# evo-design/evo

Hardware: AMD Instinct MI355X
Metric: nucleotides/sec forward scoring, evo-1 7B (higher is better)
Workload: dtype bf16; 1 GPU; evo-1-8k-base scoring, batch 8 x 8,192 nt per GPU (BASELINE configs[1]); batch_per_gpu=8, nt=8192, parallelism=single GPU

## Files before the change

### evo_amd/_build.py

```python
from __future__ import annotations

import os
import shutil
import subprocess
from pathlib import Path

ROOT = Path(__file__).resolve().parent
CSRC = ROOT / "csrc"
LIBDIR = ROOT / "_lib"
LIBNAME = os.environ.get("EVO_AMD_LIBNAME", "libevo_mi355x.so")
ARCH = "gfx950"

EXPORTS = [
    "evo_abi_version", "evo_embed_bf16", "evo_rmsnorm_bf16", "evo_hyena_seg_state", "evo_hyena_carry_scan", "evo_hyena_carry_add",
    "evo_hyena_apply", "evo_hyena_step", "evo_rope_qk_bf16", "evo_attn_fwd_causal_bf16", "evo_attn_decode_bf16",
    "evo_linear_small_m_bf16", "evo_mlp_gate_small_m_bf16", "evo_norm_mlp_gate_small_m_bf16", "evo_norm_linear_small_m_bf16", "evo_hyena_decode_fused_small_m", "evo_linear_mfma_bf16", "evo_mlp_gate_mfma_bf16", "evo_linear_xblk_mfma_bf16", "evo_hyena_ct", "evo_linear_t_mfma_bf16", "evo_rmsnorm_rows_bf16", "evo_gelu_gate_bf16",
    "evo_logprob_entropy", "evo_unembed_logprob_bf16", "evo_unembed_profile_bf16", "evo_rope_append_decode_bf16",
    "evo_linear_mfma_nf_bf16", "evo_linear_xblk_mfma_nf_bf16", "evo_mlp_gate_mfma_nf_bf16", "evo_linear_t_mfma_nf_bf16", "evo_rms_finalize_f32",
    "evo_probe_copy_f4", "evo_probe_mfma_bf16", "evo_pool_rows_bf16", "evo_sample_rows_f32",
    "evo_attn_fwd_prefix_bf16", "evo_attn_prefix_vt_bf16", "evo_attn_decode_prefix_bf16", "evo_rope_append_decode_at_bf16",
    "evo_hyena_state_at_zt",
]


def lib_path() -> Path:
    return LIBDIR / LIBNAME


def sources():
    return sorted(CSRC.glob("*.hip"))


def _hipcc() -> str:
    for cand in (os.environ.get("HIPCC"), shutil.which("hipcc"), "/opt/rocm/bin/hipcc"):
        if cand and os.path.exists(cand):
            return cand
    raise RuntimeError("hipcc not found: cannot build libevo_mi355x.so")


def is_stale() -> bool:
    out = lib_path()
    if not out.exists():
        return True
    deps = list(sources()) + list(CSRC.glob("*.h")) + [ROOT.parent / "include" / "evo_mi355x.h"]
    newest = max(p.stat().st_mtime for p in deps if p.exists())
    return newest > out.stat().st_mtime


FILE_FLAGS = {"attn_w64.hip": ["-fno-slp-vectorize", "-Wno-unused-value"]}


def _compile_one(args):
    src, obj, verbose = args
    cmd = [_hipcc(), f"--offload-arch={ARCH}", "-O3", "-std=c++17", "-fPIC", "-fno-gpu-rdc", "-Wno-inline-asm"] \
# ... 37 lines not shown
```

### evo_amd/ops.py

```python
from __future__ import annotations

import ctypes
import math
import os
import threading
from typing import Optional, Tuple

import torch

from . import _build

_c = ctypes
_PTR = _c.c_void_p
_I64 = _c.c_int64
_F32 = _c.c_float

_SIGNATURES = {
    "evo_abi_version": ([], _c.c_int),
    "evo_embed_bf16": ([_PTR, _PTR, _PTR, _I64, _I64, _I64, _PTR, _PTR], _c.c_int),
    "evo_rmsnorm_bf16": ([_PTR, _PTR, _PTR, _PTR, _I64, _I64, _F32, _PTR], _c.c_int),
    "evo_hyena_seg_state": ([_PTR, _PTR, _PTR, _PTR, _PTR, _PTR, _PTR, _I64, _I64, _I64, _I64, _I64, _PTR], _c.c_int),
    "evo_hyena_carry_scan": ([_PTR, _PTR, _PTR, _PTR, _I64, _I64, _I64, _I64, _PTR], _c.c_int),
    "evo_hyena_carry_add": ([_PTR, _PTR, _PTR, _I64, _I64, _I64, _I64, _PTR], _c.c_int),
    "evo_hyena_apply": ([_PTR] * 10 + [_I64] * 5 + [_PTR], _c.c_int),
# ... 1 lines not shown
    "evo_rope_qk_bf16": ([_PTR, _PTR, _PTR, _I64, _I64, _I64, _I64, _F32, _PTR], _c.c_int),
    "evo_attn_fwd_causal_bf16": ([_PTR] * 4 + [_I64] * 14 + [_F32, _PTR, _PTR], _c.c_int),
    "evo_attn_fwd_prefix_bf16": ([_PTR] * 6 + [_I64] * 16 + [_F32, _PTR, _PTR], _c.c_int),
    "evo_attn_prefix_vt_bf16": ([_PTR] * 2 + [_I64] * 5 + [_PTR], _c.c_int),
    "evo_attn_decode_bf16": ([_PTR] * 4 + [_I64] * 11 + [_PTR] * 3 + [_I64, _F32, _PTR], _c.c_int),
    "evo_linear_small_m_bf16": ([_PTR] * 5 + [_I64] * 3 + [_PTR, _I64, _PTR], _c.c_int),
    "evo_linear_mfma_bf16": ([_PTR] * 5 + [_I64] * 3 + [_PTR], _c.c_int),
    "evo_mlp_gate_mfma_bf16": ([_PTR] * 3 + [_I64] * 3 + [_PTR], _c.c_int),
    "evo_hyena_ct": ([_PTR] * 9 + [_I64] * 13 + [_PTR], _c.c_int),
    "evo_linear_t_mfma_bf16": ([_PTR] * 4 + [_I64] * 3 + [_PTR], _c.c_int),
    "evo_rmsnorm_rows_bf16": ([_PTR, _PTR, _PTR, _PTR, _I64, _I64, _F32, _I64, _I64, _I64, _I64, _PTR], _c.c_int),
    "evo_linear_xblk_mfma_bf16": ([_PTR] * 5 + [_I64] * 3 + [_PTR], _c.c_int),
    "evo_linear_mfma_nf_bf16": ([_PTR] * 7 + [_I64] * 4 + [_PTR], _c.c_int),
    "evo_linear_xblk_mfma_nf_bf16": ([_PTR] * 6 + [_I64] * 4 + [_PTR], _c.c_int),
    "evo_mlp_gate_mfma_nf_bf16": ([_PTR] * 4 + [_I64] * 3 + [_PTR], _c.c_int),
    "evo_linear_t_mfma_nf_bf16": ([_PTR] * 5 + [_I64] * 6 + [_PTR], _c.c_int),
    "evo_rms_finalize_f32": ([_PTR, _I64, _I64, _PTR, _I64, _I64, _I64, _F32, _PTR, _PTR], _c.c_int),
    "evo_probe_copy_f4": ([_PTR, _PTR, _I64, _PTR], _c.c_int),
    "evo_probe_mfma_bf16": ([_PTR, _I64, _I64, _PTR], _c.c_int),
    "evo_mlp_gate_small_m_bf16": ([_PTR] * 3 + [_I64] * 4 + [_PTR], _c.c_int),
    "evo_norm_linear_small_m_bf16": ([_PTR] * 5 + [_I64] * 3 + [_c.c_float, _PTR], _c.c_int),
    "evo_norm_mlp_gate_small_m_bf16": ([_PTR] * 4 + [_I64] * 3 + [_c.c_float, _I64, _PTR], _c.c_int),
    "evo_hyena_decode_fused_small_m": ([_PTR] * 12 + [_I64] * 3 + [_c.c_float, _PTR], _c.c_int),
    "evo_gelu_gate_bf16": ([_PTR, _PTR, _I64, _I64, _PTR], _c.c_int),
    "evo_logprob_entropy": ([_PTR, _I64, _PTR, _PTR, _PTR, _I64, _I64, _PTR], _c.c_int),
    "evo_unembed_logprob_bf16": ([_PTR] * 5 + [_I64] * 3 + [_PTR], _c.c_int),
    "evo_unembed_profile_bf16": ([_PTR] * 3 + [_c.POINTER(_c.c_int32), _I64] + [_PTR] * 3 + [_I64] * 3 + [_PTR], _c.c_int),
    "evo_rope_append_decode_bf16": ([_PTR] * 4 + [_F32] + [_I64] * 7 + [_F32, _PTR], _c.c_int),
    "evo_pool_rows_bf16": ([_PTR, _I64, _I64, _I64, _PTR, _I64, _PTR, _F32, _I64, _I64, _PTR, _PTR, _PTR], _c.c_int),
    "evo_attn_decode_prefix_bf16": ([_PTR] * 4 + [_I64] * 11 + [_PTR] * 3 + [_I64] * 8 + [_PTR] * 4 + [_I64, _I64, _F32, _PTR], _c.c_int),
    "evo_rope_append_decode_at_bf16": ([_PTR] * 4 + [_F32] + [_I64] * 7 + [_F32, _PTR, _PTR], _c.c_int),
    "evo_hyena_state_at_zt": ([_PTR] * 8 + [_I64] * 8 + [_PTR], _c.c_int),
    "evo_sample_rows_f32": ([_PTR, _I64, _I64, _PTR, _PTR, _PTR, _PTR, _c.c_uint64] + [_PTR] * 7 + [_I64] * 3 + [_PTR], _c.c_int),
}

_LIB = None
ABI_VERSION = 16
ATTN_GROUP_ROWS = 8


HYENA_RAGGED_SEG = 256


class EvoLibraryError(RuntimeError):
    pass


def load_library(build_if_missing: bool = True) -> ctypes.CDLL:
    global _LIB
    if _LIB is not None:
        return _LIB
    path = _build.lib_path()
    if (not path.exists() or (_build.is_stale() and os.environ.get("EVO_AMD_NO_REBUILD") != "1")) and build_if_missing:
        try:
            _build.build()
        except Exception as e:
            if not path.exists():
                raise EvoLibraryError(f"libevo_mi355x.so is missing and could not be built: {e}") from e
            import warnings
            warnings.warn(f"{path} is older than its sources and the rebuild failed ({e}); loading the stale library "
                          f"(its ABI version is checked below)")
    if not path.exists():
        raise EvoLibraryError(f"{path} not found; run `python -c 'import __graft_entry__ as g; g.build()'`")
    lib = ctypes.CDLL(str(path))
    for name, (argtypes, restype) in _SIGNATURES.items():
        fn = getattr(lib, name, None)
        if fn is None:
            raise EvoLibraryError(f"{path} does not export {name}")
        fn.argtypes = argtypes
        fn.restype = restype
# ... 45 lines not shown

    def span(self, name):
        return KernelTimer._Span(self, name)

    def summary(self):
        return {k: (len(v), sum(a.elapsed_time(b) for a, b in v) / len(v)) for k, v in self.pairs.items()}


class _NoSpan:
    def __enter__(self):
        return None

    def __exit__(self, *exc):
        return False


_NOSPAN = _NoSpan()


class HipOps:

    name = "hip-gfx950"

    def __init__(self):
        self.lib = load_library()
        if not torch.cuda.is_available():
            raise EvoLibraryError("HipOps needs a ROCm GPU (torch.cuda.is_available() is False)")
        self.seg_len_override = int(os.environ.get("EVO_AMD_SEG_LEN", "0"))
        self.attn_gemm_mfma = True
        self.attn_w64 = True
        self.fuse_norm = True
        self.attn_prescale = True
        self.hyena_tail_split = True
        self.gate_small_m_mfma = True
        self.hyena_table_guard = True
        self.all_gemm_mfma = True
        self.mlp_gate_fused = True
        self.timer: Optional[KernelTimer] = None
        self.validate_ids = os.environ.get("EVO_AMD_VALIDATE_IDS", "1") != "0"
        self.hyena_mfma = True
        self.hyena_ct_flag = True
        self._xpad = threading.local()
        self.last_hyena_io = {}

    def _t(self, name):
        return self.timer.span(name) if self.timer is not None else _NOSPAN

    PTR_ALIGN = 16

    @staticmethod
    def _align_of(dtype) -> int:
        return HipOps.PTR_ALIGN if (dtype.is_floating_point or dtype.is_complex) else torch.empty(0, dtype=dtype).element_size()

    @staticmethod
    def _check_address(addr: int, what: str, align: int = 16) -> None:
        if addr % align:
            raise RuntimeError(f"{what}: address 0x{addr:x} is not {align}-byte aligned (include/evo_mi355x.h, Conventions)")

    @staticmethod
    def _need(t: torch.Tensor, dtype, what: str):
        if not t.is_cuda:
            raise RuntimeError(f"{what}: tensor is on {t.device}; the HIP path has no CPU fallback")
        if t.dtype != dtype:
            raise RuntimeError(f"{what}: expected {dtype}, got {t.dtype}")
        if not t.is_contiguous():
            raise RuntimeError(f"{what}: tensor must be contiguous")
# ... 190 lines not shown
        Tm, Tp, Mp, r = self.zt_layout(B, T)
        K = xp.shape[1]
        N = w.shape[0]
        assert xp.shape[0] >= Mp + B * r
        zt = torch.empty(Mp // 256 + (1 if r and tail else 0), N, 256, dtype=torch.bfloat16, device=xp.device)
        self._launch("gemm_zt", "evo_linear_t_mfma_bf16", xp.data_ptr(), w.data_ptr(), _ptr(b), zt.data_ptr(), Mp, N, K)
        if r and tail:
            self._zt_tail_fill(zt, self._linear_small_m(xp[Mp:Mp + B * r], w, b, None), B, r)
        return zt

    @staticmethod
    def _zt_tail_fill(zt: torch.Tensor, z_tail: torch.Tensor, B: int, r: int) -> None:
        N = zt.shape[1]
        zt[-1].zero_()
        zt[-1].view(N, 32, 8)[:, :B, :r] = z_tail.view(B, r, N).permute(2, 0, 1)

    @staticmethod
    def zt_rows(zt: torch.Tensor, B: int, T: int, t0: int, n: int) -> torch.Tensor:
        bb = torch.arange(B, device=zt.device)[:, None].expand(B, n)
        tt = torch.arange(t0, t0 + n, device=zt.device)[None, :].expand(B, n)
        pos = HipOps.zt_positions(B, T, bb, tt).reshape(-1)
        return zt[pos // 256, :, pos % 256].view(B, n, zt.shape[1])

    @staticmethod
    def zt_from_rows(z: torch.Tensor, B: int, T: int, pad_value: float = 0.0) -> torch.Tensor:
        Tm, Tp, Mp, r = HipOps.zt_layout(B, T)
        C = z.shape[-1]
        P = Mp + (256 if r else 0)
        flat = torch.full((C, P), pad_value, dtype=z.dtype, device=z.device)
        flat[:, :B * Tp].view(C, B, Tp)[:, :, :Tm] = z[:, :Tm].permute(2, 0, 1)
        if r:
            flat[:, Mp:].view(C, 32, 8)[:, :B, :r] = z[:, Tm:].permute(2, 0, 1)
        return flat.view(C, P // 256, 256).permute(1, 0, 2).contiguous()

    def hyena_ct(self, zt, B, T, fir_w, fir_b, table, n_heads, z_halo=None, s0=None, want_state=False, poles=None,
                 state_only=False, b_first=0, y_blk=None, y_row0=0, b_total=None, main_only=False):
        self._need(zt, torch.bfloat16, "hyena z^T")
        assert zt.dim() == 3 and zt.shape[2] == 256
        D3, P = zt.shape[1], zt.shape[0] * 256
        D = D3 // 3
        Tm, Tp, Mp, r = self.zt_layout(b_first + B if b_total is None else b_total, T)
        assert D3 == 3 * D and (b_first + B) * Tp <= Mp
        if main_only:
            assert r > 0 and P in (Mp, Mp + 256) and z_halo is None and s0 is None and not state_only
        else:
            assert P == Mp + (256 if r else 0)
        T_run = Tm if main_only else T
        if table.dtype != torch.int32 or tuple(table.shape) != (D, 52, 64) or not table.is_contiguous() or not table.is_cuda:
            raise RuntimeError("hyena_ct: table must be the contiguous int32 [D, 52, 64] tensor of mfma_operand_table")
        for t, nm in ((fir_w, "fir_w"), (fir_b, "fir_b")):
            self._need(t, torch.bfloat16, "hyena " + nm)
        if z_halo is not None:
            self._need(z_halo, torch.bfloat16, "hyena z_halo")
            assert z_halo.shape == (B, 2, 3 * D)
        s0r = None
        if s0 is not None:
            s0r = torch.view_as_real(s0.to(torch.complex64).contiguous())
            assert s0r.shape == (B, D, 8, 2) and s0r.is_cuda
        s_fin = None
        if want_state or state_only:
            if poles is None:
                raise RuntimeError("hyena_ct: the end state needs the poles")
            self._need(poles, torch.float32, "hyena poles")
            assert tuple(poles.shape) == (D, 8, 2)
            s_fin = torch.empty(B, D, 8, 2, dtype=torch.float32, device=zt.device)
        yb_rows = 0
# ... 693 lines not shown
```

### evo_amd/scoring.py

```python
from typing import List, NamedTuple, Sequence, Tuple, Union

import numpy as np
import torch

from .tokenizer import CharLevelTokenizer


def prepare_batch(seqs: List[str], tokenizer: CharLevelTokenizer, prepend_bos: bool = True,
                  device: str = "cuda:0") -> Tuple[torch.Tensor, List[int]]:
    seq_lengths = [len(s) for s in seqs]
    longest = max(seq_lengths)
    bos = int(prepend_bos)
    rows = [np.frombuffer(seq.encode(), dtype=np.uint8) for seq in seqs]
    widths = {bos + r.size + (longest - n) for r, n in zip(rows, seq_lengths)}
    if len(widths) != 1:
        raise RuntimeError("prepare_batch: rows have different token lengths (non-ASCII input?)")
    width = widths.pop()
    ids = np.full((len(seqs), width), tokenizer.pad_id, dtype=np.int64)
    if prepend_bos:
        ids[:, 0] = tokenizer.eod_id
    for i, r in enumerate(rows):
        ids[i, bos:bos + r.size] = r
    return torch.from_numpy(ids).to(device), seq_lengths


def _ops_for(t: torch.Tensor):
    from .ops import default_ops
    return default_ops()


def logits_to_logprobs(logits: torch.Tensor, input_ids: torch.Tensor, trim_bos: bool = True,
                       bf16_logprobs: bool = False) -> torch.Tensor:
    if trim_bos:
        logits = logits[:, :-1]
        input_ids = input_ids[:, 1:]
    assert logits.shape[1] == input_ids.shape[1]
    B, L, V = logits.shape
    if logits.is_cuda:
        lg = logits.reshape(B * L, V)
        if lg.dtype not in (torch.bfloat16, torch.float32):
            lg = lg.float()
        lp, _ = _ops_for(lg).logprob_entropy(lg.contiguous(), input_ids.reshape(-1).to(lg.device))
        out = lp.view(B, L)
    else:
        out = torch.log_softmax(logits.float(), dim=-1).gather(2, input_ids.unsqueeze(-1).long()).squeeze(-1)
    return out.to(torch.bfloat16) if bf16_logprobs else out


def _fused_tail_ok(model, input_ids) -> bool:
    ops = getattr(model, "ops", None) if hasattr(model, "hidden_states") else None
    if not getattr(model, "has_own_unembed", True) or not isinstance(getattr(getattr(model, "unembed", None), "weight", None), torch.Tensor):
        return False
    return (ops is not None and getattr(ops, "name", "") == "hip-gfx950" and hasattr(ops, "unembed_logprob")
            and ops.unembed_logprob_ok(model.unembed.weight.new_empty(1, model.hidden_size), model.unembed.weight))


def score_logprobs_device(model, input_ids: torch.Tensor, want_entropy: bool = False):
    B, T = input_ids.shape
    if _fused_tail_ok(model, input_ids):
        with torch.no_grad():
            hid = model.hidden_states(input_ids)
            tgt = torch.full((B, T), -1, dtype=torch.int64, device=hid.device)
            tgt[:, :-1] = input_ids[:, 1:].to(hid.device)
            lp, en = model.ops.unembed_logprob(hid, model.unembed.weight, tgt.reshape(-1),
                                               want_logprob=not want_entropy, want_entropy=want_entropy)
        return (None if lp is None else lp.view(B, T)[:, :-1]), (None if en is None else en.view(B, T)[:, :-1])
    logits, _ = model(input_ids)
    if not want_entropy:
        return logits_to_logprobs(logits, input_ids, trim_bos=True), None
    logits = logits[:, :-1]
    L, V = logits.shape[1], logits.shape[2]
    if logits.is_cuda:
        lg = logits.reshape(B * L, V).contiguous()
        _, ent = _ops_for(lg).logprob_entropy(lg, None, want_logprob=False, want_entropy=True)
        return None, ent.view(B, L)
    lsm = torch.log_softmax(logits.float(), dim=-1)
    return None, -(lsm.exp() * lsm).sum(-1)


def _reduce(logprobs: np.ndarray, seq_lengths: List[int], reduce_method: str) -> List[float]:
    if reduce_method == "mean":
        fn = np.mean
    elif reduce_method == "sum":
        fn = np.sum
    else:
        raise ValueError(f"Invalid reduce_method {reduce_method}")
    return [fn(logprobs[i][: seq_lengths[i]]) for i in range(len(seq_lengths))]


def score_sequences(seqs: List[str], model, tokenizer: CharLevelTokenizer, reduce_method: str = "mean",
                    device: str = "cuda:0") -> List[float]:
    if reduce_method not in ("mean", "sum"):
        raise ValueError(f"Invalid reduce_method {reduce_method}")
    input_ids, seq_lengths = prepare_batch(seqs, tokenizer, device=device, prepend_bos=True)
# ... 26 lines not shown


def profile_token_ids(tokens: Union[str, Sequence[int]] = "ACGT", vocab: int = 512) -> Tuple[int, ...]:
    if isinstance(tokens, (str, bytes)):
        raw = tokens.encode("utf-8") if isinstance(tokens, str) else tokens
        if isinstance(tokens, str) and len(raw) != len(tokens):
            raise ValueError(f"tokens: {tokens!r} holds a non-ASCII character (one character must be one byte id)")
        ids = list(raw)
    else:
        if isinstance(tokens, torch.Tensor):
            tokens = tokens.tolist()
        try:
            tokens = list(tokens)
            ids = [int(t) for t in tokens]
        except (TypeError, ValueError) as e:
            raise ValueError(f"tokens: expected an ASCII string or a sequence of ints, got {tokens!r}") from e
        if any(i != t for i, t in zip(ids, tokens)):
            raise ValueError(f"tokens: expected integer ids, got {tokens!r}")
    if not 1 <= len(ids) <= PROFILE_MAX_TOKENS:
        raise ValueError(f"tokens: expected 1 to {PROFILE_MAX_TOKENS} tokens, got {len(ids)}")
    for i in ids:
        if not 0 <= i < vocab:
            raise ValueError(f"tokens: id {i} is outside [0, {vocab})")
    if len(set(ids)) != len(ids):
        raise ValueError(f"tokens: a token is given twice in {tokens!r}")
    return tuple(ids)


def score_profile_device(model, input_ids: torch.Tensor, token_ids):
    ids = profile_token_ids(token_ids)
    B, T = input_ids.shape
    if _fused_tail_ok(model, input_ids) and hasattr(model.ops, "unembed_profile"):
        with torch.no_grad():
            hid = model.hidden_states(input_ids)
            tgt = torch.full((B, T), -1, dtype=torch.int64, device=hid.device)
            tgt[:, :-1] = input_ids[:, 1:].to(hid.device)
            sl, lp, en = model.ops.unembed_profile(hid, model.unembed.weight, ids, tgt.reshape(-1))
        return lp.view(B, T)[:, :-1], en.view(B, T)[:, :-1], sl.view(B, T, len(ids))[:, :-1]
    with torch.no_grad():
        logits, _ = model(input_ids)
        lsm = torch.log_softmax(logits[:, :-1].float(), dim=-1)
        lp = lsm.gather(2, input_ids[:, 1:].to(lsm.device).unsqueeze(-1).long()).squeeze(-1)
        en = -(lsm.exp() * lsm).sum(-1)
        sl = lsm.index_select(2, torch.tensor(ids, dtype=torch.int64, device=lsm.device))
    return lp, en, sl


def position_profiles(seqs: List[str], model, tokenizer: CharLevelTokenizer, tokens: Union[str, Sequence[int]] = "ACGT",
                      device: str = "cuda:0") -> List[PositionProfile]:
    ids = profile_token_ids(tokens)
    if len(seqs) == 0:
        raise ValueError("position_profiles: no sequences")
    input_ids, seq_lengths = prepare_batch(seqs, tokenizer, device=device, prepend_bos=True)
    with torch.inference_mode():
        lp, en, sl = score_profile_device(model, input_ids, ids)
    lp, en, sl = lp.float().cpu().numpy(), en.float().cpu().numpy(), sl.float().cpu().numpy()
    out = [PositionProfile(lp[i][:n].copy(), en[i][:n].copy(), sl[i][:n].copy(), ids) for i, n in enumerate(seq_lengths)]
    assert all(len(s) == len(p.logprob) for s, p in zip(seqs, out))
    return out


def substitution_scores(profile: PositionProfile) -> np.ndarray:
    return profile.token_logprobs - profile.logprob[:, None]


def predicted_tokens(profile: PositionProfile) -> np.ndarray:
    return np.asarray(profile.tokens, dtype=np.int64)[profile.token_logprobs.argmax(-1)]
# ... 203 lines not shown
```

### evo_amd/sh/model.py

```python
from __future__ import annotations

import math
import weakref
from typing import Dict, List, Optional, Tuple

import torch
import torch.nn as nn

from ..ops import HipOps
from .cache import InferenceParams, RecurrentInferenceParams
from .utils import dotdict


def _cfg(config, key, default):
    v = config.get(key, None) if isinstance(config, dict) else getattr(config, key, None)
    return default if v is None else v


class _Params(nn.Module):

    def __init__(self, **shapes):
        super().__init__()
        for name, (shape, dtype) in shapes.items():
            self.register_parameter(name, nn.Parameter(torch.empty(*shape, dtype=dtype), requires_grad=False))
# ... 422 lines not shown
            a = ops.mlp_gate(n2, blk.mlp._w12, w12g=blk.mlp._w12g)
        ops.linear_residual_(x2d, a, blk.mlp._w3)

    def _mfma_hyena_ok(self, B: int, T: int) -> bool:
        ops = self.ops
        D, H = self.hidden_size, self.num_heads
        if not getattr(ops, "hyena_mfma", False) or not hasattr(ops, "hyena_ct") or D != H * 128:
            return False
        return T >= 32 and B * T >= 256

    def _mfma_table(self, blk):
        f = blk.filter
        if getattr(f, "_mfma_tab", None) is None or f._mfma_tab.device != blk.projections.weight.device:
            from ..hyena_tables import mfma_operand_table
            f._mfma_tab = mfma_operand_table(f._poles, f._residues, f.D.data)
        return f._mfma_tab

    def _table_ok(self, blk) -> bool:
        f = blk.filter
        if not getattr(self.ops, "hyena_table_guard", True):
            return True
        if getattr(f, "_tab_prec", None) is None:
            from ..hyena_tables import table_precision
            f._tab_prec = float(table_precision(f._poles, f._residues, f.D.data).max())
        from ..hyena_tables import TABLE_TOL
        return f._tab_prec <= TABLE_TOL

    def _hyena_ct_ok(self, x2d, blk, B, T) -> bool:
        ops = self.ops
        w = blk.projections.weight
        return (getattr(ops, "hyena_ct_flag", False) and hasattr(ops, "hyena_ct") and x2d.is_cuda and w.dtype == torch.bfloat16
                and w.is_contiguous() and ops.zt_shape_ok(B, T, w.shape[0], w.shape[1]))

    def _hyena_block(self, i, blk, x2d, B, T, cache: Optional[RecurrentInferenceParams], mask=None, rs=None):
        ops = self.ops
        D, H = self.hidden_size, self.num_heads
        f = blk.filter
        have_state = cache is not None and i in cache.fir_state_dict
        K1 = self.short_filter_length - 1
        lens = getattr(cache, "lengths", None) if cache is not None and T > 1 else None
        if lens is not None and (have_state or mask is not None):
            raise ValueError("a ragged prefill (lengths) starts at t = 0 without a padding mask: no resumed prefill, no mask")
        if have_state and T == 1:
            y = ops.hyena_decode_fused(x2d, blk.pre_norm.scale, self.eps, blk.projections.weight, blk.projections.bias,
                                       cache.fir_state_dict[i], cache.state_dict[i], f._fir_w, f.short_filter_bias,
                                       f._poles, f._residues, f.D, H)
        elif mask is None and self._mfma_hyena_ok(B, T) and self._hyena_ct_ok(x2d, blk, B, T) and self._table_ok(blk):
            table = self._mfma_table(blk)
            nf = self._nf_ok(B * T, mask)
            pb = None if blk.projections.bias is None else blk.projections.bias.data
            Tm, _, _, r_tail = ops.zt_layout(B, T)
            split = (cache is None and r_tail == 1 and getattr(ops, "hyena_tail_split", False) and HipOps.fused_rows_ok(B, D)
                     and pb is not None)
            if nf and rs is not None and ops.zt_stream_rows_ok(B, T):
                wp_f = self._folded(blk, "_wp_f", blk.projections.weight, blk.pre_norm.scale)
                zt = ops.linear_t_rs(x2d, rs, wp_f, pb, blk.projections.weight.data, blk.pre_norm.scale, self.eps, B, T, tail=not split)
            else:
                xp = ops.rmsnorm_rows(x2d, blk.pre_norm.scale, self.eps, B, T)
                zt = ops.linear_t(xp, blk.projections.weight.data, pb, B, T, tail=not split)
            yb = ops.yblk_empty(B * T, D, zt.device)
            if split:
                y, state = ops.hyena_ct(zt, B, T, f._fir_w, f.short_filter_bias, table, H, want_state=True, poles=f._poles, y_blk=yb,
                                        main_only=True)
                ix = self._tail_split_index(B, T, zt.device)
                fir = zt[ix["zblk"], :, 256 - K1:].contiguous()
                x_tail = x2d.view(B, T, D)[:, Tm].contiguous()
                y_tail = ops.hyena_decode_fused(x_tail, blk.pre_norm.scale, self.eps, blk.projections.weight, blk.projections.bias, fir, state,
                                                f._fir_w, f.short_filter_bias, f._poles, f._residues, f.D, H)
                yb[ix["yblk"], :, ix["yrow"], :] = y_tail.view(B, D // 16, 16)
            elif cache is None:
                y = ops.hyena_ct(zt, B, T, f._fir_w, f.short_filter_bias, table, H, y_blk=yb)
            elif lens is not None:
                y = ops.hyena_ct(zt, B, T, f._fir_w, f.short_filter_bias, table, H, y_blk=yb)
                cache.state_dict[i], cache.fir_state_dict[i] = ops.hyena_state_at_zt(zt, B, T, lens, f._fir_w, f.short_filter_bias, f._poles, H)
            else:
                halo = s0 = None
                if have_state:
                    halo = cache.fir_state_dict[i].transpose(1, 2).contiguous()
                    s0 = cache.state_dict[i]
                y, state = ops.hyena_ct(zt, B, T, f._fir_w, f.short_filter_bias, table, H, z_halo=halo, s0=s0,
                                        want_state=True, poles=f._poles, y_blk=yb)
                cache.fir_state_dict[i] = ops.zt_rows(zt, B, T, T - K1, K1).transpose(1, 2).contiguous()
                cache.state_dict[i] = state
            if nf:
                return self._mlp_residual_rs_(blk, x2d, self._mixer_out_rs_(blk, x2d, y, blk.out_filter_dense.weight, blk.out_filter_dense.bias))
            self._mlp_residual_(blk, x2d, self._mixer_out_(blk, x2d, y, blk.out_filter_dense.weight, blk.out_filter_dense.bias), None)
            return None
        else:
            z = ops.norm_linear(x2d, blk.pre_norm.scale, self.eps, blk.projections.weight, blk.projections.bias)
            if mask is not None:
                z.mul_(mask[0])
            z3 = z.view(B, T, 3 * D)
            halo = s0 = None
            if have_state:
                halo = cache.fir_state_dict[i].transpose(1, 2).contiguous()
                s0 = cache.state_dict[i]
            kw = {} if mask is None else {"mask": mask[1]}
            y3, state = ops.hyena_prefill(z3, f._fir_w, f.short_filter_bias, f._poles, f._residues, f.D, H,
                                          z_halo=halo, s0=s0, want_state=cache is not None and lens is None, **kw)
            y = y3.view(B * T, D)
            if lens is not None:
                cache.state_dict[i], cache.fir_state_dict[i] = ops.hyena_state_at(z3, lens, f._fir_w, f.short_filter_bias, f._poles, H)
            elif cache is not None:
                tail = z3[:, -K1:, :]
                if halo is not None and T < K1:
                    tail = torch.cat([halo[:, T:], tail], dim=1)
                elif T < K1:
                    tail = torch.cat([z3.new_zeros(B, K1 - T, 3 * D), tail], dim=1)
                cache.fir_state_dict[i] = tail.transpose(1, 2).contiguous()
                cache.state_dict[i] = state
        self._mlp_residual_(blk, x2d, self._mixer_out_(blk, x2d, y, blk.out_filter_dense.weight, blk.out_filter_dense.bias),
                            None if mask is None else mask[0])
        return None

    def _tail_split_index(self, B: int, T: int, device):
        key = (B, T, str(device))
        cur = getattr(self, "_tail_ix", None)
        if cur is None or cur[0] != key:
            Tm = self.ops.zt_layout(B, T)[0]
            b = torch.arange(B, device=device)
            R = b * T + Tm
            cur = (key, {"zblk": (b * Tm + Tm - 1) // 256, "yblk": R // self.ops.YBLK, "yrow": R % self.ops.YBLK})
            self._tail_ix = cur
        return cur[1]

    def _kv_buffer(self, cache: InferenceParams, i: int, B: int, need: int, like: torch.Tensor):
        H, hd = self.num_heads, self.head_dim
        kv = cache.key_value_memory_dict.get(i)
        cap_b = max(int(cache.max_batch_size or 1), B)
        if kv is None or kv.shape[0] < B or kv.shape[1] < need or kv.device != like.device:
            cap_t = max(int(cache.max_seqlen or 0), need)
            if kv is not None and kv.shape[1] < need:
                cap_t = max(cap_t, 2 * kv.shape[1])
            new = torch.zeros(cap_b, cap_t, 2, H, hd, dtype=like.dtype, device=like.device)
            if kv is not None:
                b0, t0 = min(kv.shape[0], cap_b), min(kv.shape[1], cap_t)
                new[:b0, :t0] = kv[:b0, :t0].to(like.device)
            cache.key_value_memory_dict[i] = kv = new
        return kv

    def _attn_block(self, i, blk, x2d, B, T, cache: Optional[InferenceParams], mask=None, rs=None):
        ops = self.ops
        D, H, hd = self.hidden_size, self.num_heads, self.head_dim
        mha = blk.inner_mha_cls
        if mask is not None:
            x2d.mul_(mask[0])
# ... 53 lines not shown
                else:
                    a = ops.attention(q, k, v, off, **ak).view(B * T, D)
        if nf:
            return self._mlp_residual_rs_(blk, x2d, self._mixer_out_rs_(blk, x2d, a, mha.out_proj.weight, mha.out_proj.bias))
        self._mlp_residual_(blk, x2d, self._mixer_out_(blk, x2d, a, mha.out_proj.weight, mha.out_proj.bias, mfma=True),
                            None if mask is None else mask[0])
        return None

    max_rows_per_pass = 160 * 1024

    def _row_groups(self, B: int, T: int):
        cap = max(1, self.max_rows_per_pass // T)

        def fits(p):
            r = (p * T) % 256
            return r == 0 or HipOps.fused_rows_ok(r, 4096)

        if B <= cap and (fits(B) or B * T < 65536):
            return [B]
        n0 = (B + cap - 1) // cap

        def split(n):
            q, r = divmod(B, n)
            return [q + 1] * r + [q] * (n - r)

        n = n0
        while n <= B and (B // n) * T >= 32768:
            g = split(n)
            if all(fits(p) for p in set(g)):
                return g
            n += 1
        return split(n0)

    def hidden_states(self, x: torch.Tensor, inference_params_dict=None, padding_mask=None) -> torch.Tensor:
        if not self._packed:
            self._pack()
        if x.dim() != 2:
            raise ValueError("input_ids must be [batch, length]")
        B, T = x.shape
        ops = self.ops
        if padding_mask is not None and tuple(padding_mask.shape) != (B, T):
            raise ValueError(f"padding_mask must be [batch, length] = {(B, T)}, got {tuple(padding_mask.shape)}")
        groups = self._row_groups(B, T) if inference_params_dict is None else [B]
        if len(groups) > 1:
            out, b0 = None, 0
            for nb in groups:
                pm = None if padding_mask is None else padding_mask[b0:b0 + nb]
                hg = self.hidden_states(x[b0:b0 + nb], None, pm)
                if out is None:
                    out = torch.empty(B * T, hg.shape[1], dtype=hg.dtype, device=hg.device)
                out[b0 * T:(b0 + nb) * T] = hg
                b0 += nb
            return out
        h = ops.embed(x.to(self.device), self.embedding_layer.weight)
        mask = None
        if padding_mask is not None:
            pm = padding_mask.to(self.device) != 0
            mask = (pm.reshape(B * T, 1).to(h.dtype), pm.to(torch.uint8).contiguous())
        mha_c = inference_params_dict["mha"] if inference_params_dict is not None else None
        hy_c = inference_params_dict["hyena"] if inference_params_dict is not None else None
        dyn = T == 1 and mha_c is not None and getattr(mha_c, "pos_tensor", None) is not None
        if dyn and not hasattr(ops, "rope_append_decode"):
            mha_c._rot_dyn = self._rotary_dyn(mha_c.pos_tensor)
        try:
            self._run_blocks(h, B, T, mha_c, hy_c, mask)
        finally:
            if dyn:
                mha_c._rot_dyn = None
        if self.norm is not None:
            h = ops.rmsnorm(h, None, self.norm.scale, self.eps)
        return h

    def _run_blocks(self, h: torch.Tensor, B: int, T: int, mha_c, hy_c, mask, stop: Optional[int] = None, after_block=None) -> None:
        stop = self.num_layers if stop is None else stop
        rs = None
        taps = getattr(self, "block_taps", None)
        tap_idxs = getattr(self, "block_tap_idxs", None)
        for i in range(stop):
            blk = self.blocks[i]
            if taps is not None and (tap_idxs is None or i in tap_idxs):
                taps.append(h.clone())
            if isinstance(blk, _AttentionBlock):
                rs = self._attn_block(i, blk, h, B, T, mha_c, mask, rs)
            else:
                rs = self._hyena_block(i, blk, h, B, T, hy_c, mask, rs)
            if after_block is not None:
                after_block(i, h)
        if stop == self.num_layers and taps is not None and (tap_idxs is None or self.num_layers in tap_idxs):
            taps.append(h.clone())

    @torch.no_grad()
    def embeddings(self, input_ids: torch.Tensor, layers, pooling: str = "mean", start: int = 1, lengths=None,
                   padding_mask=None, inference_params_dict=None) -> Dict:
        from ..embeddings import check_pooling, normalize_layers
        if padding_mask is not None:
            raise ValueError("embeddings: padding_mask is not supported (pass the true lengths instead: pads are never pooled)")
        if inference_params_dict is not None:
            raise ValueError("embeddings: an inference cache is not supported (embeddings are a stateless forward)")
        if not self.embedding_layer.weight.is_cuda:
            raise RuntimeError(f"embeddings: the model's weights are on {self.embedding_layer.weight.device}; move the model to the GPU")
        layers = normalize_layers(layers, self.num_layers)
        check_pooling(pooling)
        if input_ids.dim() != 2:
            raise ValueError("input_ids must be [batch, length]")
        B, T = input_ids.shape
        if lengths is None:
            lengths = [T - start] * B
        lengths = [int(n) for n in lengths]
        if len(lengths) != B:
            raise ValueError(f"embeddings: {len(lengths)} lengths for a batch of {B}")
        if start < 0 or any(n < 1 or start + n > T for n in lengths):
            raise ValueError(f"embeddings: every row needs 1 <= length and start + length <= T = {T} (start {start}, lengths {lengths})")
        if not self._packed:
            self._pack()
        ops = self.ops
        D = self.hidden_size
        dev = self.device
        blocks = [l for l in layers if l != "final"]
# ... 166 lines not shown
```

### include/evo_mi355x.h

```cpp
#ifndef EVO_MI355X_H
#define EVO_MI355X_H

#include <stdint.h>

#ifdef __cplusplus
extern "C" {
#endif

#define EVO_ABI_VERSION 16
int evo_abi_version(void);

int evo_embed_bf16(const int64_t* ids, const void* weight, void* out,
                   int64_t n_tok, int64_t D, int64_t vocab, int* bad_flag, void* stream);

int evo_rmsnorm_bf16(void* x, const void* bias, const void* scale, void* out,
                     int64_t M, int64_t D, float eps, void* stream);

int evo_hyena_seg_state(const void* z, const void* z_halo, const void* fir_w, const void* fir_b,
                        const float* poles, float* agg, const uint8_t* mask,
                        int64_t B, int64_t T, int64_t D, int64_t n_heads, int64_t seg_len, void* stream);
int evo_hyena_carry_scan(float* agg, const float* poles, const float* s0, float* s_final,
                         int64_t B, int64_t T, int64_t D, int64_t seg_len, void* stream);
int evo_hyena_carry_add(float* agg, const float* poles, const float* s0,
                        int64_t B, int64_t T, int64_t D, int64_t seg_len, void* stream);
int evo_hyena_apply(const void* z, const void* z_halo, const void* fir_w, const void* fir_b,
                    const float* poles, const float* residues, const void* dskip,
                    const float* agg, void* y, const uint8_t* mask,
                    int64_t B, int64_t T, int64_t D, int64_t n_heads, int64_t seg_len, void* stream);

int evo_hyena_ct(const void* zt, const void* z_halo, const void* fir_w, const void* fir_b, const void* table, void* y,
                 const float* s0, float* s_out, const float* poles, int64_t B, int64_t T, int64_t D, int64_t n_heads,
                 int64_t zt_pitch, int64_t row_pitch, int64_t zt_row0, int64_t tail_T, int64_t tail_pos0, int64_t state_only,
                 int64_t y_blocked_rows, int64_t y_row0, int64_t y_row_pitch, void* stream);

#define EVO_HYENA_RAGGED_SEG 256
int evo_hyena_state_at_zt(const void* zt, const int64_t* lens, const void* fir_w, const void* fir_b, const float* poles,
                          float* s_out, void* fir_out, float* ws, int64_t ws_bytes,
                          int64_t B, int64_t T, int64_t D, int64_t n_heads,
                          int64_t zt_pitch, int64_t row_pitch, int64_t zt_row0, void* stream);

int evo_linear_xblk_mfma_bf16(const void* x_blk, const void* w, const void* bias, const void* residual, void* y,
                              int64_t M, int64_t N, int64_t K, void* stream);

int evo_linear_t_mfma_bf16(const void* x, const void* w, const void* bias, void* zt, int64_t Mp, int64_t N, int64_t K, void* stream);

int evo_rmsnorm_rows_bf16(void* x, const void* bias, const void* scale, void* out, int64_t M, int64_t D, float eps,
                          int64_t T, int64_t Tp, int64_t Tm, int64_t tail0, void* stream);

int evo_hyena_step(const void* z_t, void* fir_state, float* iir_state,
                   const void* fir_w, const void* fir_b, const float* poles, const float* residues,
                   const void* dskip, void* y, int64_t B, int64_t D, int64_t n_heads, void* stream);

int evo_rope_qk_bf16(void* qkv, const float* cos_t, const float* sin_t,
                     int64_t B, int64_t T, int64_t H, int64_t hd, float q_scale, void* stream);

int evo_rope_append_decode_bf16(void* qkv, void* kv, const int64_t* pos, const float* inv_freq, float scaling,
                                int64_t B, int64_t H, int64_t hd, int64_t kv_sb, int64_t kv_st, int64_t kv_sw, int64_t kv_sh,
                                float q_scale, void* stream);
int evo_rope_append_decode_at_bf16(void* qkv, void* kv, const int64_t* pos, const float* inv_freq, float scaling,
                                   int64_t B, int64_t H, int64_t hd, int64_t kv_sb, int64_t kv_st, int64_t kv_sw, int64_t kv_sh,
                                   float q_scale, const int64_t* widx, void* stream);

int evo_attn_fwd_causal_bf16(const void* q, const void* k, const void* v, void* o,
                             int64_t B, int64_t H, int64_t Tq, int64_t Tk, int64_t q_pos0,
                             int64_t q_sb, int64_t q_st, int64_t q_sh,
                             int64_t k_sb, int64_t k_st, int64_t k_sh,
                             int64_t v_sb, int64_t v_st, int64_t v_sh,
                             float softmax_scale, void* vt_ws, void* stream);

int evo_attn_fwd_prefix_bf16(const void* q, const void* k, const void* v, const void* k_pre, const void* vt_pre, void* o,
                             int64_t B, int64_t H, int64_t Tq, int64_t P,
                             int64_t q_sb, int64_t q_st, int64_t q_sh,
                             int64_t k_sb, int64_t k_st, int64_t k_sh,
                             int64_t v_sb, int64_t v_st, int64_t v_sh,
                             int64_t kp_st, int64_t kp_sh, int64_t vtp_row,
                             float softmax_scale, void* vt_ws, void* stream);
int evo_attn_prefix_vt_bf16(const void* v_pre, void* vt_pre, int64_t P, int64_t H, int64_t vp_st, int64_t vp_sh, int64_t vt_row,
                            void* stream);

int evo_attn_decode_bf16(const void* q, const void* k, const void* v, void* o,
// ... 80 lines not shown
```

Baseline: 107,500 nt/s.

## Replace block-0 projection GEMM with a gather from a per-vocab precomputed table

Block 0's input is the token embedding, so rmsnorm followed by the input projection depends only on the token id. The scoring path now runs rmsnorm and projection over the whole vocabulary (V rows) and then gathers the per-token z^T rows into the blocked layout with a new HIP kernel, skipping the large M=B*T projection GEMM in the first Hyena block. The table is rebuilt on every call, but V is tiny for nucleotides, so the cost is mainly the gather's memory traffic. It applies only to unmasked, cache-free scoring and plain or tail-split zt layouts.

New measurement: 108,000 nt/s, median of 6. No clear change (+0.5%).

```diff
diff --git a/evo_amd/_build.py b/evo_amd/_build.py
--- a/evo_amd/_build.py
+++ b/evo_amd/_build.py
@@ -19,7 +19,7 @@
     "evo_linear_mfma_nf_bf16", "evo_linear_xblk_mfma_nf_bf16", "evo_mlp_gate_mfma_nf_bf16", "evo_linear_t_mfma_nf_bf16", "evo_rms_finalize_f32",
     "evo_probe_copy_f4", "evo_probe_mfma_bf16", "evo_pool_rows_bf16", "evo_sample_rows_f32",
     "evo_attn_fwd_prefix_bf16", "evo_attn_prefix_vt_bf16", "evo_attn_decode_prefix_bf16", "evo_rope_append_decode_at_bf16",
-    "evo_hyena_state_at_zt",
+    "evo_hyena_state_at_zt", "evo_zt_from_table_bf16",
 ]
 
 
diff --git a/evo_amd/csrc/zt_table.hip b/evo_amd/csrc/zt_table.hip
--- /dev/null
+++ b/evo_amd/csrc/zt_table.hip
@@ -0,0 +1,61 @@
+#include "common.h"
+#include "../../include/evo_mi355x.h"
+
+#define ZG_BLK 256
+#define ZG_THREADS 256
+#define ZG_CPI (ZG_THREADS / 32)
+#define ZG_STRIP 64
+
+typedef uint32_t zg_u32x4 __attribute__((ext_vector_type(4)));
+
+__global__ __launch_bounds__(ZG_THREADS) void zt_from_table_kernel(
+    const int64_t* __restrict__ ids, const uint16_t* __restrict__ table, const uint16_t* __restrict__ bias, uint16_t* __restrict__ zt,
+    int B, int T_used, int64_t Tp, int64_t ids_pitch, int N, int V) {
+    const int grp = threadIdx.x & 31;
+    const int sub = threadIdx.x >> 5;
+    const int64_t p0 = (int64_t)blockIdx.x * ZG_BLK + grp * 8;
+    const int64_t b = p0 / Tp;
+    const int64_t t0 = p0 - b * Tp;
+    int off[8];
+#pragma unroll
+    for (int j = 0; j < 8; ++j) {
+        off[j] = -1;
+        if (b < B && t0 + j < T_used) {
+            const int64_t v = ids[b * ids_pitch + t0 + j];
+            if (v >= 0 && v < V) off[j] = (int)((v >> 8) * (int64_t)N * ZG_BLK + (v & 255));
+        }
+    }
+    const int c0 = blockIdx.y * ZG_STRIP;
+    const int c1 = c0 + ZG_STRIP < N ? c0 + ZG_STRIP : N;
+    uint16_t* __restrict__ dst = zt + (int64_t)blockIdx.x * N * ZG_BLK + grp * 8;
+#pragma unroll 2
+    for (int c = c0 + sub; c < c1; c += ZG_CPI) {
+        const uint16_t* __restrict__ row = table + (int64_t)c * ZG_BLK;
+        const uint32_t pad = bias ? bias[c] : 0u;
+        uint32_t e[8];
+#pragma unroll
+        for (int j = 0; j < 8; ++j) e[j] = off[j] >= 0 ? (uint32_t)row[off[j]] : pad;
+        zg_u32x4 w;
+        w.x = e[0] | (e[1] << 16);
+        w.y = e[2] | (e[3] << 16);
+        w.z = e[4] | (e[5] << 16);
+        w.w = e[6] | (e[7] << 16);
+        *(zg_u32x4*)(dst + (int64_t)c * ZG_BLK) = w;
+    }
+}
+
+extern "C" int evo_zt_from_table_bf16(const int64_t* ids, const void* table, const void* bias, void* zt, int64_t B, int64_t T_used,
+                                      int64_t ids_pitch, int64_t Tp, int64_t Mp, int64_t N, int64_t V, void* stream) {
+    if (B <= 0 || T_used <= 0 || Tp <= 0 || Mp <= 0 || N <= 0 || V <= 0) return -1;
+    if (N % 8 != 0 || V % ZG_BLK != 0 || Mp % ZG_BLK != 0 || Tp % 8 != 0) return -1;
+    if (T_used > Tp || ids_pitch < T_used || B > Mp / Tp || B * Tp > Mp) return -1;
+    if (!ids || !table || !zt) return -1;
+    if (((uintptr_t)ids & 7) != 0 || ((uintptr_t)table & 15) != 0 || ((uintptr_t)zt & 15) != 0 || ((uintptr_t)bias & 1) != 0) return -1;
+    if (V > 0x7fffffffll / N / 2 || Mp > 0xfffffff0ll / N / 2) return -1;
+    if (B > 0x7fffffffll || T_used > 0x7fffffffll) return -1;
+    const int64_t strips = (N + ZG_STRIP - 1) / ZG_STRIP;
+    if (strips > 65535) return -1;
+    hipLaunchKernelGGL(zt_from_table_kernel, dim3((unsigned)(Mp / ZG_BLK), (unsigned)strips), dim3(ZG_THREADS), 0, (hipStream_t)stream,
+                       ids, (const uint16_t*)table, (const uint16_t*)bias, (uint16_t*)zt, (int)B, (int)T_used, Tp, ids_pitch, (int)N, (int)V);
+    return evo_launch_status();
+}
diff --git a/evo_amd/ops.py b/evo_amd/ops.py
--- a/evo_amd/ops.py
+++ b/evo_amd/ops.py
@@ -57,10 +57,11 @@
     "evo_rope_append_decode_at_bf16": ([_PTR] * 4 + [_F32] + [_I64] * 7 + [_F32, _PTR, _PTR], _c.c_int),
     "evo_hyena_state_at_zt": ([_PTR] * 8 + [_I64] * 8 + [_PTR], _c.c_int),
     "evo_sample_rows_f32": ([_PTR, _I64, _I64, _PTR, _PTR, _PTR, _PTR, _c.c_uint64] + [_PTR] * 7 + [_I64] * 3 + [_PTR], _c.c_int),
+    "evo_zt_from_table_bf16": ([_PTR] * 4 + [_I64] * 7 + [_PTR], _c.c_int),
 }
 
 _LIB = None
-ABI_VERSION = 16
+ABI_VERSION = 17
 ATTN_GROUP_ROWS = 8
 
 
@@ -172,6 +173,7 @@
         self.fuse_norm = True
         self.attn_prescale = True
         self.hyena_tail_split = True
+        self.block0_table = True
         self.gate_small_m_mfma = True
         self.hyena_table_guard = True
         self.all_gemm_mfma = True
@@ -428,6 +430,22 @@
         if r:
             flat[:, Mp:].view(C, 32, 8)[:, :B, :r] = z[:, Tm:].permute(2, 0, 1)
         return flat.view(C, P // 256, 256).permute(1, 0, 2).contiguous()
+
+    def zt_from_table(self, table: torch.Tensor, ids: torch.Tensor, B: int, T_used: int, bias: Optional[torch.Tensor] = None) -> torch.Tensor:
+        self._need(table, torch.bfloat16, "zt_from_table table")
+        if bias is not None:
+            self._need(bias, torch.bfloat16, "zt_from_table bias")
+        if not ids.is_cuda or ids.dtype != torch.int64 or ids.dim() != 2 or ids.shape[0] != B or ids.shape[1] < T_used or (ids.shape[1] > 1 and ids.stride(1) != 1):
+            raise RuntimeError(f"zt_from_table ids: expected a device int64 matrix [{B}, >= {T_used}] with unit column stride")
+        self._check_address(ids.data_ptr(), "zt_from_table ids", 8)
+        Tm, Tp, Mp, r = self.zt_layout(B, T_used)
+        if r:
+            raise RuntimeError(f"zt_from_table: {B} x {T_used} takes the tail form of zt_layout (only the plain form is gathered)")
+        nvb, N, _ = table.shape
+        zt = torch.empty(Mp // 256, N, 256, dtype=torch.bfloat16, device=table.device)
+        self._launch("zt_table", "evo_zt_from_table_bf16", ids.data_ptr(), table.data_ptr(), _ptr(bias), zt.data_ptr(), B, T_used,
+                     ids.stride(0) if B > 1 else max(ids.shape[1], T_used), Tp, Mp, N, nvb * 256)
+        return zt
 
     def hyena_ct(self, zt, B, T, fir_w, fir_b, table, n_heads, z_halo=None, s0=None, want_state=False, poles=None,
                  state_only=False, b_first=0, y_blk=None, y_row0=0, b_total=None, main_only=False):
diff --git a/evo_amd/scoring.py b/evo_amd/scoring.py
--- a/evo_amd/scoring.py
+++ b/evo_amd/scoring.py
@@ -55,11 +55,15 @@
             and ops.unembed_logprob_ok(model.unembed.weight.new_empty(1, model.hidden_size), model.unembed.weight))
 
 
+def _scoring_hidden_states(model, input_ids: torch.Tensor) -> torch.Tensor:
+    return getattr(model, "scoring_hidden_states", model.hidden_states)(input_ids)
+
+
 def score_logprobs_device(model, input_ids: torch.Tensor, want_entropy: bool = False):
     B, T = input_ids.shape
     if _fused_tail_ok(model, input_ids):
         with torch.no_grad():
-            hid = model.hidden_states(input_ids)
+            hid = _scoring_hidden_states(model, input_ids)
             tgt = torch.full((B, T), -1, dtype=torch.int64, device=hid.device)
             tgt[:, :-1] = input_ids[:, 1:].to(hid.device)
             lp, en = model.ops.unembed_logprob(hid, model.unembed.weight, tgt.reshape(-1),
@@ -152,7 +156,7 @@
     B, T = input_ids.shape
     if _fused_tail_ok(model, input_ids) and hasattr(model.ops, "unembed_profile"):
         with torch.no_grad():
-            hid = model.hidden_states(input_ids)
+            hid = _scoring_hidden_states(model, input_ids)
             tgt = torch.full((B, T), -1, dtype=torch.int64, device=hid.device)
             tgt[:, :-1] = input_ids[:, 1:].to(hid.device)
             sl, lp, en = model.ops.unembed_profile(hid, model.unembed.weight, ids, tgt.reshape(-1))
diff --git a/evo_amd/sh/model.py b/evo_amd/sh/model.py
--- a/evo_amd/sh/model.py
+++ b/evo_amd/sh/model.py
@@ -478,7 +478,7 @@
         return (getattr(ops, "hyena_ct_flag", False) and hasattr(ops, "hyena_ct") and x2d.is_cuda and w.dtype == torch.bfloat16
                 and w.is_contiguous() and ops.zt_shape_ok(B, T, w.shape[0], w.shape[1]))
 
-    def _hyena_block(self, i, blk, x2d, B, T, cache: Optional[RecurrentInferenceParams], mask=None, rs=None):
+    def _hyena_block(self, i, blk, x2d, B, T, cache: Optional[RecurrentInferenceParams], mask=None, rs=None, zt0=None):
         ops = self.ops
         D, H = self.hidden_size, self.num_heads
         f = blk.filter
@@ -495,10 +495,11 @@
             table = self._mfma_table(blk)
             nf = self._nf_ok(B * T, mask)
             pb = None if blk.projections.bias is None else blk.projections.bias.data
-            Tm, _, _, r_tail = ops.zt_layout(B, T)
-            split = (cache is None and r_tail == 1 and getattr(ops, "hyena_tail_split", False) and HipOps.fused_rows_ok(B, D)
-                     and pb is not None)
-            if nf and rs is not None and ops.zt_stream_rows_ok(B, T):
+            Tm = ops.zt_layout(B, T)[0]
+            split = self._tail_split_ok(B, T, cache, pb)
+            if zt0 is not None:
+                zt = zt0
+            elif nf and rs is not None and ops.zt_stream_rows_ok(B, T):
                 wp_f = self._folded(blk, "_wp_f", blk.projections.weight, blk.pre_norm.scale)
                 zt = ops.linear_t_rs(x2d, rs, wp_f, pb, blk.projections.weight.data, blk.pre_norm.scale, self.eps, B, T, tail=not split)
             else:
@@ -558,6 +559,11 @@
         self._mlp_residual_(blk, x2d, self._mixer_out_(blk, x2d, y, blk.out_filter_dense.weight, blk.out_filter_dense.bias),
                             None if mask is None else mask[0])
         return None
+
+    def _tail_split_ok(self, B: int, T: int, cache, pb) -> bool:
+        ops = self.ops
+        return (cache is None and ops.zt_layout(B, T)[3] == 1 and getattr(ops, "hyena_tail_split", False)
+                and HipOps.fused_rows_ok(B, self.hidden_size) and pb is not None)
 
     def _tail_split_index(self, B: int, T: int, device):
         key = (B, T, str(device))
@@ -677,7 +683,7 @@
             n += 1
         return split(n0)
 
-    def hidden_states(self, x: torch.Tensor, inference_params_dict=None, padding_mask=None) -> torch.Tensor:
+    def hidden_states(self, x: torch.Tensor, inference_params_dict=None, padding_mask=None, scoring: bool = False) -> torch.Tensor:
         if not self._packed:
             self._pack()
         if x.dim() != 2:
@@ -691,13 +697,14 @@
             out, b0 = None, 0
             for nb in groups:
                 pm = None if padding_mask is None else padding_mask[b0:b0 + nb]
-                hg = self.hidden_states(x[b0:b0 + nb], None, pm)
+                hg = self.hidden_states(x[b0:b0 + nb], None, pm, scoring)
                 if out is None:
                     out = torch.empty(B * T, hg.shape[1], dtype=hg.dtype, device=hg.device)
                 out[b0 * T:(b0 + nb) * T] = hg
                 b0 += nb
             return out
-        h = ops.embed(x.to(self.device), self.embedding_layer.weight)
+        x = x.to(self.device)
+        h = ops.embed(x, self.embedding_layer.weight)
         mask = None
         if padding_mask is not None:
             pm = padding_mask.to(self.device) != 0
@@ -707,8 +714,9 @@
         dyn = T == 1 and mha_c is not None and getattr(mha_c, "pos_tensor", None) is not None
         if dyn and not hasattr(ops, "rope_append_decode"):
             mha_c._rot_dyn = self._rotary_dyn(mha_c.pos_tensor)
+        zt0 = self._block0_zt(x, B, T, h) if scoring and mask is None and inference_params_dict is None else None
         try:
-            self._run_blocks(h, B, T, mha_c, hy_c, mask)
+            self._run_blocks(h, B, T, mha_c, hy_c, mask, zt0=zt0)
         finally:
             if dyn:
                 mha_c._rot_dyn = None
@@ -716,7 +724,28 @@
             h = ops.rmsnorm(h, None, self.norm.scale, self.eps)
         return h
 
-    def _run_blocks(self, h: torch.Tensor, B: int, T: int, mha_c, hy_c, mask, stop: Optional[int] = None, after_block=None) -> None:
+    def scoring_hidden_states(self, x: torch.Tensor) -> torch.Tensor:
+        return self.hidden_states(x, scoring=True)
+
+    def _block0_zt(self, ids: torch.Tensor, B: int, T: int, h: torch.Tensor) -> Optional[torch.Tensor]:
+        ops = self.ops
+        blk = self.blocks[0]
+        if not (getattr(ops, "block0_table", False) and hasattr(ops, "zt_from_table") and isinstance(blk, _HyenaBlock)):
+            return None
+        if not (self._mfma_hyena_ok(B, T) and self._hyena_ct_ok(h, blk, B, T) and self._table_ok(blk)):
+            return None
+        emb = self.embedding_layer.weight.data
+        V, D = emb.shape
+        pb = None if blk.projections.bias is None else blk.projections.bias.data
+        Tm, _, _, r = ops.zt_layout(B, T)
+        if r != 0 and not self._tail_split_ok(B, T, None, pb):
+            return None
+        if V % 256 != 0 or not ops.zt_shape_ok(1, V, 3 * D, D) or not HipOps._bf16_ok(emb, scale=blk.pre_norm.scale):
+            return None
+        table = ops.linear_t(ops.rmsnorm(emb, None, blk.pre_norm.scale, self.eps), blk.projections.weight.data, pb, 1, V)
+        return ops.zt_from_table(table, ids if ids.dtype == torch.int64 else ids.long(), B, Tm, pb)
+
+    def _run_blocks(self, h: torch.Tensor, B: int, T: int, mha_c, hy_c, mask, stop: Optional[int] = None, after_block=None, zt0=None) -> None:
         stop = self.num_layers if stop is None else stop
         rs = None
         taps = getattr(self, "block_taps", None)
@@ -728,7 +757,7 @@
             if isinstance(blk, _AttentionBlock):
                 rs = self._attn_block(i, blk, h, B, T, mha_c, mask, rs)
             else:
-                rs = self._hyena_block(i, blk, h, B, T, hy_c, mask, rs)
+                rs = self._hyena_block(i, blk, h, B, T, hy_c, mask, rs, zt0 if i == 0 else None)
             if after_block is not None:
                 after_block(i, h)
         if stop == self.num_layers and taps is not None and (tap_idxs is None or self.num_layers in tap_idxs):
diff --git a/include/evo_mi355x.h b/include/evo_mi355x.h
--- a/include/evo_mi355x.h
+++ b/include/evo_mi355x.h
@@ -7,7 +7,7 @@
 extern "C" {
 #endif
 
-#define EVO_ABI_VERSION 16
+#define EVO_ABI_VERSION 17
 int evo_abi_version(void);
 
 int evo_embed_bf16(const int64_t* ids, const void* weight, void* out,
@@ -46,6 +46,9 @@
 
 int evo_rmsnorm_rows_bf16(void* x, const void* bias, const void* scale, void* out, int64_t M, int64_t D, float eps,
                           int64_t T, int64_t Tp, int64_t Tm, int64_t tail0, void* stream);
+
+int evo_zt_from_table_bf16(const int64_t* ids, const void* table, const void* bias, void* zt, int64_t B, int64_t T_used,
+                           int64_t ids_pitch, int64_t Tp, int64_t Mp, int64_t N, int64_t V, void* stream);
 
 int evo_hyena_step(const void* z_t, void* fir_state, float* iir_state,
                    const void* fir_w, const void* fir_b, const float* poles, const float* residues,
```
